# ruc-aimc-lab/GeoFormer

Measured on AMD Instinct MI355X. Metric: image-pairs/sec (640x640), higher is better.
Workload: dtype f16

## Files before the change

geoformer_amd/_lib.py:

```python
import ctypes
import os

_HERE = os.path.dirname(os.path.abspath(__file__))
LIB_PATH = os.environ.get('GF_LIB_PATH') or os.path.join(_HERE, 'libgeoformer_hip.so')

GF_F32, GF_F16, GF_BF16 = 0, 1, 2
GF_IMAGE_U8, GF_IMAGE_F32_NORMALISED, GF_IMAGE_F32_NORMALISED_RCP = 0, 1, 2

c_void_p, c_int, c_float, c_size_t = ctypes.c_void_p, ctypes.c_int, ctypes.c_float, ctypes.c_size_t
c_long, c_uint32 = ctypes.c_long, ctypes.c_uint32

SIGNATURES = {
    'gf_abi_version': (c_int, []),
    'gf_last_error': (ctypes.c_char_p, []),
    'gf_profile_filter': (None, [ctypes.c_char_p]),
    'gf_profile_enable': (None, [c_int]),
    'gf_profile_collect': (c_int, [ctypes.c_char_p, ctypes.POINTER(ctypes.c_double), ctypes.POINTER(c_int),
                                   ctypes.POINTER(ctypes.c_double)]),
    'gf_dual_softmax_workspace_bytes': (c_size_t, [c_int, c_int, c_int]),
    'gf_dual_softmax_match_only_supported': (c_int, [c_int, c_int, c_int, c_int, c_int, c_int]),
    'gf_dual_softmax_conf_at': (c_int, [c_void_p, c_void_p, c_int, c_int, c_int, c_int, c_int, c_float, c_void_p, c_void_p, c_void_p, c_int,
                                        c_void_p, c_void_p, c_size_t, c_void_p]),
    'gf_dual_softmax_match': (c_int, [c_void_p, c_void_p, c_int, c_int, c_int, c_int, c_int, c_void_p, c_void_p,
                                      c_float, c_float, c_int, c_int, c_int, c_float, c_void_p, c_void_p, c_void_p,
# ... 37 lines not shown
    'gf_encoder_kv_state': (c_int, [c_void_p, c_long, c_int, c_int, c_int, c_void_p, c_void_p, c_void_p, c_void_p, c_size_t, c_void_p]),
    'gf_encoder_layer': (c_int, [c_void_p, c_long, c_void_p, c_long, c_void_p, c_int, c_void_p, c_float, c_void_p, c_void_p, c_float,
                                 c_float, c_int, c_void_p, c_int, c_void_p, c_long, c_int, c_int, c_int, c_void_p]),
    'gf_encoder_layer_kv': (c_int, [c_void_p, c_long, c_void_p, c_int, c_void_p, c_float, c_void_p, c_void_p, c_float, c_float, c_int,
                                    c_void_p, c_long, c_int, c_int, c_int, c_void_p, c_int, c_void_p, c_void_p, c_size_t, c_void_p]),
    'gf_fine_layer': (c_int, [c_void_p, c_void_p, c_void_p, c_int, c_int, c_int, c_void_p, c_void_p, c_float, c_float, c_float, c_void_p]),
    'gf_conv3x3_supported': (c_int, [c_int, c_int]),
    'gf_conv3x3s2_supported': (c_int, [c_int, c_int]),
    'gf_lateral_supported': (c_int, [c_int, c_int]),
    'gf_lateral_upsample_add_nhwc': (c_int, [c_void_p, c_void_p, c_void_p, c_void_p, c_int, c_int, c_int, c_int, c_int, c_int, c_int, c_int, c_void_p]),
    'gf_conv3x3_nhwc': (c_int, [c_void_p, c_void_p, c_void_p, c_void_p, c_void_p, c_void_p, c_int, c_int, c_int, c_int, c_int, c_int,
                                c_float, c_int, c_void_p]),
    'gf_linear': (c_int, [c_void_p, c_long, c_int, c_void_p, c_long, c_int, c_void_p, c_void_p, c_void_p, c_int, c_int,
                          c_void_p, c_void_p, c_float, c_void_p, c_long, c_void_p, c_int, c_void_p, c_long, c_int, c_int,
                          c_int, c_void_p]),
    'gf_ransac_workspace_bytes': (c_size_t, [c_int, c_int]),
    'gf_ransac_homography': (c_int, [c_void_p, c_void_p, c_void_p, c_int, c_int, c_float, c_void_p, c_void_p, c_float,
                                     c_int, c_uint32, c_int, c_int, c_void_p, c_void_p, c_void_p, c_void_p, c_void_p, c_void_p,
                                     c_void_p, c_void_p, c_size_t, c_void_p]),
    'gf_ransac_homography_v2': (c_int, [c_void_p, c_void_p, c_void_p, c_int, c_int, c_float, c_void_p, c_void_p, c_float,
                                        c_int, c_uint32, c_int, c_int, c_void_p, c_void_p, c_void_p, c_void_p, c_void_p, c_void_p,
                                        c_void_p, c_void_p, c_size_t, c_void_p, c_int]),
    'gf_window_geometry': (c_int, [c_void_p, c_void_p, c_int, c_int, c_int, c_int, c_int, c_int, c_int, c_int,
                                   c_void_p, c_void_p, c_void_p, c_void_p, c_void_p]),
    'gf_inlier_index': (c_int, [c_void_p, c_void_p, c_void_p, c_void_p, c_int, c_int, c_int, c_int, c_int, c_int,
                                c_void_p, c_void_p, c_void_p, c_void_p, c_void_p, c_void_p]),
    'gf_self_attention_workspace_bytes': (c_size_t, [c_int, c_int, c_int]),
    'gf_self_attention_gathered': (c_int, [c_void_p, c_void_p, c_void_p, c_int, c_int, c_int, c_int, c_int, c_long,
                                           c_long, c_long, c_void_p, c_long, c_void_p, c_int, c_void_p, c_void_p,
                                           c_size_t, c_void_p]),
# ... 63 lines not shown
```

geoformer_amd/csrc/gf_common.h:

```cpp
#pragma once
#include <hip/hip_runtime.h>
#include <stdint.h>
#include <stdio.h>

#include "../../include/geoformer_hip.h"

typedef float v16f __attribute__((ext_vector_type(16)));
typedef float v4f __attribute__((ext_vector_type(4)));
typedef _Float16 v8h __attribute__((ext_vector_type(8)));
typedef _Float16 v4h __attribute__((ext_vector_type(4)));
typedef _Float16 v2h __attribute__((ext_vector_type(2)));
typedef uint32_t v4u __attribute__((ext_vector_type(4)));
typedef __bf16 gf_bf16;
typedef gf_bf16 v8b __attribute__((ext_vector_type(8)));
typedef gf_bf16 v4b __attribute__((ext_vector_type(4)));
template <typename T, int N>
using gf_vec = T __attribute__((ext_vector_type(N)));
typedef short gf_v4s __attribute__((__vector_size__(4 * sizeof(short))));

void gf_set_error(const char* fmt, ...);

#define GF_CHECK_ARG(cond, msg)                                   \
    do {                                                          \
        if (!(cond)) {                                            \
// ... 56 lines not shown
    static constexpr int kPer16B = 8;
};

__device__ __forceinline__ float gf_to_float(float x) { return x; }
__device__ __forceinline__ float gf_to_float(_Float16 x) { return (float)x; }
__device__ __forceinline__ float gf_to_float(gf_bf16 x) { return (float)x; }
template <typename T>
__device__ __forceinline__ T gf_from_float(float x);
template <>
__device__ __forceinline__ float gf_from_float<float>(float x) { return x; }
template <>
__device__ __forceinline__ _Float16 gf_from_float<_Float16>(float x) { return (_Float16)x; }
template <>
__device__ __forceinline__ gf_bf16 gf_from_float<gf_bf16>(float x) { return (gf_bf16)x; }

template <typename T>
struct Mma32;
template <>
struct Mma32<float> {
    using Frag = v4f;
    static constexpr int kGroup = 8;
    static __device__ __forceinline__ void mma(const Frag& a, const Frag& b, v16f& c) {
        c = __builtin_amdgcn_mfma_f32_32x32x2f32(a.x, b.x, c, 0, 0, 0);
        c = __builtin_amdgcn_mfma_f32_32x32x2f32(a.y, b.y, c, 0, 0, 0);
        c = __builtin_amdgcn_mfma_f32_32x32x2f32(a.z, b.z, c, 0, 0, 0);
        c = __builtin_amdgcn_mfma_f32_32x32x2f32(a.w, b.w, c, 0, 0, 0);
    }
};
template <>
struct Mma32<_Float16> {
// ... 138 lines not shown
```

geoformer_amd/csrc/k3_linear.hip:

```cpp
#include <math.h>

#include <type_traits>

#include "gf_common.h"

#ifndef K3_TRACE
#define K3_TRACE 0
#endif
#if K3_TRACE
__device__ long long k3_trace[1024 * 4 * 16];
#define K3_T(slot) do { if (lane == 0 && blockIdx.y == 0 && blockIdx.x < 1024) k3_trace[(blockIdx.x * 4 + wave) * 16 + (slot)] = clock64(); } while (0)
extern "C" int gf_debug_k3_trace(long long* out) {
    return (int)hipMemcpyFromSymbol(out, HIP_SYMBOL(k3_trace), sizeof(long long) * 1024 * 4 * 16);
}
#else
#define K3_T(slot)
#endif

namespace {

enum { EPI_NONE = 0, EPI_RELU = 1, EPI_TANH = 2, EPI_LN = 3, EPI_LN_RES = 4, EPI_UPADD = 5 };

struct LinArgs {
    const void* a1;
    const void* a2;
    long lda1, lda2;
    int k1, k2;
    const void* w;
    const float* bias;
    const void* rgbias;
    int rg_rows;
    const float* gamma;
    const float* beta;
    float eps;
    const void* res;
    long ldres;
    const int32_t* flag;
    int flag_rows;
    void* out;
    long ldo;
    int M, N;
    const void* up_lo;
    int up_h, up_w, up_H, up_W, up_n;
    float up_ry, up_rx;
    int rm_w;
    long rm_line, rm_pix;
};

__device__ __forceinline__ void lin_tile(int& row_tile, int& col_tile) {
    const int gx = gridDim.x, gy = gridDim.y;
    row_tile = blockIdx.x;
    col_tile = blockIdx.y;
    if (gy > 1 && (gx & 7) == 0) {
        const int id = blockIdx.y * gx + blockIdx.x, grp = id / (8 * gy), j = id - grp * (8 * gy);
        row_tile = grp * 8 + (j & 7);
        col_tile = j >> 3;
    }
}

template <typename T, int NB, int EPI, bool CONVX = false>
__global__ __launch_bounds__(256, sizeof(T) == 2 ? 2 : 1) void linear_kernel(LinArgs a) {
    using Mm = Mma32<T>;
    using Frag = typename Mm::Frag;
    constexpr int EPC = 16 / sizeof(T);
    constexpr int BK = 128 / sizeof(T);
    constexpr int WROWS = 32 * NB;
    constexpr int ROWS = 128 + WROWS;
    constexpr int NLD = ROWS * 8 / 256;
    extern __shared__ __attribute__((aligned(16))) char smem[];
    char* st = smem;
    char* sw = smem + 128 * 128;
    float* vec = reinterpret_cast<float*>(smem + ROWS * 128);
    const int tid = threadIdx.x, lane = tid & 63, wave = tid >> 6, h = lane >> 5, lr = lane & 31;
    int row_tile, col_tile;
    lin_tile(row_tile, col_tile);
    const int m0 = row_tile * 128, n0 = col_tile * WROWS;
    const int K = a.k1 + a.k2;
// ... 9 lines not shown
    int dst[NLD];
    bool isa[NLD];
#pragma unroll
    for (int p = 0; p < NLD; ++p) {
        const int e = p * 256 + tid, row = e >> 3, c = e & 7;
        isa[p] = row < 128;
        if (isa[p]) {
            src[p] = nullptr;
            dst[p] = gf_lds_off(row, c);
        } else {
            const int wr = row - 128;
            src[p] = (const T*)a.w + (size_t)min(n0 + wr, a.N - 1) * K + c * EPC;
            dst[p] = 128 * 128 + gf_lds_off(wr, c);
        }
    }
    v4u regs[NLD];
    const bool ragged = CONVX && (K % BK) != 0;
    auto gload = [&](int k0) {
        const bool first = k0 < a.k1;
        const T* ab = (const T*)(first ? a.a1 : a.a2);
        const long ld = first ? a.lda1 : a.lda2;
        const int kk = first ? k0 : k0 - a.k1;
#pragma unroll
        for (int p = 0; p < NLD; ++p) {
            const int e = p * 256 + tid, row = e >> 3, c = e & 7;
            const T* g;
            if (isa[p]) {
                const int r = min(m0 + row, a.M - 1);
                const size_t ro = (CONVX && a.rm_w > 0) ? (size_t)(r / a.rm_w) * a.rm_line + (size_t)(r % a.rm_w) * a.rm_pix : (size_t)r * ld;
                g = ab + ro + kk + c * EPC;
            } else {
                g = src[p] + k0;
            }
            if (!ragged || k0 + c * EPC < K) regs[p] = *reinterpret_cast<const v4u*>(g);
            else regs[p] = v4u{0u, 0u, 0u, 0u};
        }
    };
    auto lstore = [&]() {
#pragma unroll
        for (int p = 0; p < NLD; ++p) *reinterpret_cast<v4u*>(smem + dst[p]) = regs[p];
    };
// ... 216 lines not shown
        for (int nb = 0; nb < NB; ++nb)
#pragma unroll
            for (int r4 = 0; r4 < 4; ++r4) {
                const int c = nb * 32 + 8 * r4 + 4 * h;
                if (n0 + c >= a.N) continue;
                v4f v{acc[nb][4 * r4], acc[nb][4 * r4 + 1], acc[nb][4 * r4 + 2], acc[nb][4 * r4 + 3]};
                if constexpr (EPI == EPI_LN_RES) {
                    const v4f x = *reinterpret_cast<const v4f*>(rp + c);
                    v = keep ? v4f{x.x + v.x, x.y + v.y, x.z + v.z, x.w + v.w} : x;
                }
                *reinterpret_cast<v4f*>(op + c) = v;
            }
    }
}

template <typename T, int EPI>
__global__ __launch_bounds__(256, 2) void linear_kernel_w2(LinArgs a) {
    using Frag = typename Mma32<T>::Frag;
    using V4 = gf_vec<T, 4>;
    using V8 = gf_vec<T, 8>;
    constexpr int EPC = 8, BK = 64, WROWS = 256, ROWS = 128 + WROWS, NLD = ROWS * 8 / 256;
    extern __shared__ __attribute__((aligned(16))) char smem[];
    char* st = smem;
    char* sw = smem + 128 * 128;
    float* vec = reinterpret_cast<float*>(smem + ROWS * 128);
    const int tid = threadIdx.x, lane = tid & 63, wave = tid >> 6, h = lane >> 5, lr = lane & 31;
    const int tm = wave >> 1, tn = wave & 1;
    int row_tile, col_tile;
    lin_tile(row_tile, col_tile);
    const int m0 = row_tile * 128, n0 = col_tile * WROWS;
    const int K = a.k1 + a.k2;
    if (tid < WROWS) vec[tid] = (a.bias && n0 + tid < a.N) ? a.bias[n0 + tid] : 0.f;
    const T* src[NLD];
    int dst[NLD];
    bool isa[NLD];
#pragma unroll
    for (int p = 0; p < NLD; ++p) {
        const int e = p * 256 + tid, row = e >> 3, c = e & 7;
        isa[p] = row < 128;
        if (isa[p]) {
            src[p] = nullptr;
            dst[p] = gf_lds_off(row, c);
        } else {
            const int wr = row - 128;
            src[p] = (const T*)a.w + (size_t)min(n0 + wr, a.N - 1) * K + c * EPC;
            dst[p] = 128 * 128 + gf_lds_off(wr, c);
        }
    }
    v4u regs[NLD];
    auto gload = [&](int k0) {
        const bool first = k0 < a.k1;
        const T* ab = (const T*)(first ? a.a1 : a.a2);
        const long ld = first ? a.lda1 : a.lda2;
        const int kk = first ? k0 : k0 - a.k1;
#pragma unroll
        for (int p = 0; p < NLD; ++p) {
            const int e = p * 256 + tid, row = e >> 3, c = e & 7;
            const T* g = isa[p] ? ab + (size_t)min(m0 + row, a.M - 1) * ld + kk + c * EPC : src[p] + k0;
            regs[p] = *reinterpret_cast<const v4u*>(g);
        }
    };
    v16f acc[2][4];
#pragma unroll
    for (int t = 0; t < 2; ++t)
#pragma unroll
        for (int nb = 0; nb < 4; ++nb)
#pragma unroll
            for (int r = 0; r < 16; ++r) acc[t][nb][r] = 0.f;
    const int nk = K / BK;
    gload(0);
    for (int kt = 0; kt < nk; ++kt) {
        __syncthreads();
// ... 33 lines not shown
    for (int t = 0; t < 2; ++t) {
#pragma unroll
        for (int nb = 0; nb < 4; ++nb)
#pragma unroll
            for (int r4 = 0; r4 < 4; ++r4) {
                const int c = nb * 32 + 8 * r4 + 4 * h;
                *reinterpret_cast<V4*>(ot + lr * RS + c * 2) =
                    V4{(T)acc[t][nb][4 * r4], (T)acc[t][nb][4 * r4 + 1], (T)acc[t][nb][4 * r4 + 2], (T)acc[t][nb][4 * r4 + 3]};
            }
        __builtin_amdgcn_fence(__ATOMIC_RELEASE, "wavefront");
        __builtin_amdgcn_wave_barrier();
        __builtin_amdgcn_fence(__ATOMIC_ACQUIRE, "wavefront");
#pragma unroll
        for (int it = 0; it < 8; ++it) {
            const int row = it * 4 + prow, tg = m0 + tm * 64 + t * 32 + row, cg = n0 + tn * 128 + pch * 8;
            if (tg >= a.M || cg >= a.N) continue;
            *reinterpret_cast<V8*>((T*)a.out + (size_t)tg * a.ldo + cg) = *reinterpret_cast<const V8*>(ot + row * RS + pch * 16);
        }
        __builtin_amdgcn_fence(__ATOMIC_RELEASE, "wavefront");
        __builtin_amdgcn_wave_barrier();
    }
}

template <typename T, int NB, int EPI, bool CONVX = false>
void lin_launch1(const LinArgs& a, hipStream_t st) {
    constexpr int WROWS = 32 * NB;
    size_t lds = (size_t)(128 + WROWS) * 128 + 3 * WROWS * sizeof(float);
    if (lds < 4 * 32 * 272) lds = 4 * 32 * 272;
    linear_kernel<T, NB, EPI, CONVX><<<dim3((a.M + 127) / 128, (a.N + WROWS - 1) / WROWS), 256, lds, st>>>(a);
}

template <typename T, int NB>
void lin_launch(const LinArgs& a, int epi, hipStream_t st) {
    switch (epi) {
        case EPI_NONE: lin_launch1<T, NB, EPI_NONE>(a, st); break;
        case EPI_RELU: lin_launch1<T, NB, EPI_RELU>(a, st); break;
        case EPI_TANH: lin_launch1<T, NB, EPI_TANH>(a, st); break;
        case EPI_LN: lin_launch1<T, NB, EPI_LN>(a, st); break;
        default: lin_launch1<T, NB, EPI_LN_RES>(a, st); break;
    }
}

}

// ... 42 lines not shown
    } else if (dtype == GF_F32) {
        if (wide) lin_launch<float, 8>(a, epilogue, st);
        else lin_launch<float, 4>(a, epilogue, st);
    } else if (dtype == GF_F16) {
        if (wide) lin_launch<_Float16, 8>(a, epilogue, st);
        else lin_launch<_Float16, 4>(a, epilogue, st);
    } else {
        if (wide) lin_launch<gf_bf16, 8>(a, epilogue, st);
        else lin_launch<gf_bf16, 4>(a, epilogue, st);
    }
    gf_prof_end("k3_linear", pt, st);
    GF_CHECK_LAUNCH();
    return GF_OK;
}

extern "C" int gf_conv1x1_upsample_add_nhwc(const void* x, const void* w, const void* lo, void* out, int N, int h, int wl,
                                            int H, int W, int Cin, int Cout, int dtype, void* stream) {
    GF_CHECK_ARG(x && w && lo && out, "null pointer");
    GF_CHECK_ARG(N > 0 && h > 0 && wl > 0 && H > 0 && W > 0, "empty problem");
    GF_CHECK_ARG(dtype == GF_F16 || dtype == GF_BF16, "built for 16-bit maps (the inference backbone)");
    GF_CHECK_ARG(Cin % 32 == 0 && Cout % 32 == 0, "Cin and Cout must be multiples of 32");
    GF_CHECK_ARG((long)N * H * W < (1l << 31), "too many pixels");
    GF_CHECK_ARG((uintptr_t)x % 16 == 0 && (uintptr_t)out % 16 == 0 && (uintptr_t)lo % 16 == 0, "tensors must be 16-byte aligned");
    LinArgs a{};
    a.a1 = x; a.lda1 = Cin; a.k1 = Cin; a.w = w; a.out = out; a.ldo = Cout; a.M = N * H * W; a.N = Cout;
    a.up_lo = lo; a.up_h = h; a.up_w = wl; a.up_H = H; a.up_W = W; a.up_n = N;
    a.up_ry = H > 1 ? (float)(h - 1) / (float)(H - 1) : 0.f;
    a.up_rx = W > 1 ? (float)(wl - 1) / (float)(W - 1) : 0.f;
    hipStream_t st = (hipStream_t)stream;
    void* pt = gf_prof_begin("k3_upadd", st, 2.0 * ((double)a.M * (Cin + Cout) + (double)N * h * wl * Cout + (double)Cin * Cout));
// ... 29 lines not shown
```

geoformer_amd/csrc/k_fine.hip:

```cpp
#include <math.h>

#include <type_traits>

#include "gf_common.h"

namespace {

struct FgArgs {
    const void* f0;
    const void* f1;
    long s0n, s0c, s0h, s0w, s1n, s1c, s1h, s1w;
    int H0, W0, H1, W1, C;
    const void* c0;
    const void* c1;
    int L, S, CC;
    const int64_t* b_ids;
    const int64_t* i_ids;
    const int64_t* j_ids;
    int M, w0c, w1c, stride, W;
    void* win;
    void* ccat;
};

template <typename TF, typename T>
// ... 6 lines not shown
    const TF* f = (const TF*)(side ? a.f1 : a.f0);
    const long sn = side ? a.s1n : a.s0n, sc = side ? a.s1c : a.s0c, sh = side ? a.s1h : a.s0h, sw = side ? a.s1w : a.s0w;
    const int cy = (cell / wc) * a.stride - a.W / 2, cx = (cell % wc) * a.stride - a.W / 2;
    T* out = (T*)a.win + ((size_t)side * a.M + m) * a.W * a.W * a.C;
    if (t < a.C) {
        for (int k = 0; k < a.W * a.W; ++k) {
            const int y = cy + k / a.W, x = cx + k % a.W;
            float v = 0.f;
            if (y >= 0 && y < Hf && x >= 0 && x < Wf) v = gf_to_float(f[b * sn + t * sc + y * sh + x * sw]);
            out[(size_t)k * a.C + t] = gf_from_float<T>(v);
        }
    }
    const T* cf = (const T*)(side ? a.c1 : a.c0) + ((size_t)b * (side ? a.S : a.L) + cell) * a.CC;
    T* co = (T*)a.ccat + ((size_t)side * a.M + m) * a.CC;
    for (int c = t; c < a.CC; c += blockDim.x) co[c] = cf[c];
}

template <typename TF, typename T>
__device__ __forceinline__ v4u fg_convert8(v4u v) {
    if constexpr (std::is_same<TF, T>::value) {
        return v;
    } else {
        const gf_vec<TF, 8> x = __builtin_bit_cast(gf_vec<TF, 8>, v);
        gf_vec<T, 8> o;
#pragma unroll
        for (int k = 0; k < 8; ++k) o[k] = gf_from_float<T>(gf_to_float(x[k]));
        return __builtin_bit_cast(v4u, o);
    }
}

template <typename TF, typename T>
__global__ __launch_bounds__(256) void fine_gather_rows(FgArgs a) {
    static_assert(sizeof(TF) == 2 && sizeof(T) == 2, "16-byte pieces of 8 elements on both sides");
    const int lane = threadIdx.x & 63, u = blockIdx.x * 4 + (threadIdx.x >> 6);
    if (u >= 2 * a.M) return;
    const int side = u >= a.M, m = side ? u - a.M : u;
    const int b = (int)a.b_ids[m];
    const int cell = (int)(side ? a.j_ids[m] : a.i_ids[m]);
    const int wc = side ? a.w1c : a.w0c;
    const int Hf = side ? a.H1 : a.H0, Wf = side ? a.W1 : a.W0;
    const TF* f = (const TF*)(side ? a.f1 : a.f0);
    const long sn = side ? a.s1n : a.s0n, sh = side ? a.s1h : a.s0h, sw = side ? a.s1w : a.s0w;
    const int cy = (cell / wc) * a.stride - a.W / 2, cx = (cell % wc) * a.stride - a.W / 2;
// ... 307 lines not shown
```

geoformer_amd/model/modules.py:

```python
import copy
import math
from typing import Dict, Optional

import torch
import torch.nn as nn
from .. import fused, ops


class PositionEncodingSine(nn.Module):

    def __init__(self, d_model, max_shape=(256, 256), temp_bug_fix=False):
        super().__init__()
        self.d_model, self.max_shape, self.temp_bug_fix = d_model, tuple(max_shape), temp_bug_fix
        self._tables = {}

    def table(self, h, w, device):
        key = (h, w, str(device))
        if key not in self._tables:
            if h > self.max_shape[0] or w > self.max_shape[1]:
                raise ValueError(f'feature map {h}x{w} exceeds max_shape {self.max_shape}')
            c = self.d_model
            ypos = torch.ones(h, w).cumsum(0).float().unsqueeze(0)
            xpos = torch.ones(h, w).cumsum(1).float().unsqueeze(0)
            k2 = torch.arange(0, c // 2, 2).float()
# ... 61 lines not shown
    def fusable_window(self, dtype, seq_len):
        return (dtype != torch.float32 and self.d_model == 128 and self.nhead == 8 and self.attention_kind == 'linear'
                and self.activation == 'relu' and seq_len <= 32)

    def invalidate(self):
        self._cache = {}

    def project_q(self, x):
        return ops.linear(x, self.weights(x.dtype)['q'])

    def project_kv(self, source):
        kv = ops.linear(source, self.weights(source.dtype)['kv'])
        c = self.d_model
        return kv[..., :c], kv[..., c:]

    def project_qkv(self, x):
        qkv = ops.linear(x, self.weights(x.dtype)['qkv'])
        c = self.d_model
        return qkv[..., :c], qkv[..., c:2 * c], qkv[..., 2 * c:]

    def finish(self, x, message, row_flag=None, flag_rows=0, out=None):
        w = self.weights(x.dtype)
        if self.fusable(x.dtype):
            return fused.encoder_layer(x, w['stream_finish'], w['ln'], self.norm1.eps, self.norm2.eps,
                                       0 if self.activation == 'relu' else 1, msg=message, row_flag=row_flag,
                                       flag_rows=flag_rows, out=out)
        act = ops.EPI_RELU if self.activation == 'relu' else ops.EPI_TANH
        message = ops.linear(message, w['merge'], epilogue=ops.EPI_LN, ln=w['n1'], eps=self.norm1.eps)
        hid = ops.linear(x, w['w1'], a2=message, epilogue=act)
        return ops.linear(hid, w['w2'], epilogue=ops.EPI_LN_RES, ln=w['n2'], eps=self.norm2.eps, residual=x,
# ... 201 lines not shown
    return out


class GeoTransformer(nn.Module):
    def __init__(self, config, layer_names, d_model, linear=True):
        super().__init__()
        if linear:
            raise NotImplementedError('GeoModule builds its transformer with linear=False (geo_module.py:20-21)')
        self.config, self.d_model, self.layer_names, self.nhead = config, d_model, layer_names, config['nhead']
        layer = LoFTREncoderLayer(d_model, self.nhead, 'full', 'tanh')
        self.layers = nn.ModuleList([copy.deepcopy(layer) for _ in self.layer_names])
        for p in self.parameters():
            if p.dim() > 1:
                nn.init.xavier_uniform_(p)
        self.norm = nn.LayerNorm(d_model)

    def forward(self, feat0, feat1, geo, both: Optional[torch.Tensor] = None):
        assert self.d_model == feat0.size(2), 'the feature number of src and transformer must be equal'
        n, L, S = feat0.shape[0], feat0.shape[1], feat1.shape[1]
        same = feat0.shape == feat1.shape
        nk = geo['nidx']
        if same:
            if both is None:
                both = torch.cat([feat0, feat1], 0)
            feat0, feat1 = both[:n], both[n:]
        for layer, name in zip(self.layers, self.layer_names):
            if name == 'self':
                if same:
                    q, k, v = layer.project_qkv(both)
                    msg = ops.self_attention_gathered(q, k, v, geo['idx_both'], geo['nidx_both'], self.nhead)
                    both = layer.finish(both, msg, geo['nidx_both'], L)
                    feat0, feat1 = both[:n], both[n:]
                else:
                    k, v = layer.project_kv(feat0)
                    m0 = ops.self_attention_gathered(layer.project_q(feat0), k, v, geo['idx0'], nk[:, 0], self.nhead)
                    k, v = layer.project_kv(feat1)
                    m1 = ops.self_attention_gathered(layer.project_q(feat1), k, v, geo['idx1'], nk[:, 1], self.nhead)
                    feat0 = layer.finish(feat0, m0, geo['nidx_t'][0], L)
                    feat1 = layer.finish(feat1, m1, geo['nidx_t'][1], S)
            elif name == 'cross':
                if same:
                    q, k, v = layer.project_qkv(both)
                    q0, q1, k0, k1, v0, v1 = q[:n], q[n:], k[:n], k[n:], v[:n], v[n:]
                else:
                    k0, v0 = layer.project_kv(feat0)
                    k1, v1 = layer.project_kv(feat1)
                    q0, q1 = layer.project_q(feat0), layer.project_q(feat1)
                m0 = ops.window_cross_attention(q0, k1, v1, geo['win1'], geo['valid'], self.nhead, geo.get('hw0'), geo.get('hw1'))
                m1 = ops.window_cross_attention(q1, k0, v0, geo['win0'], geo['valid'], self.nhead, geo.get('hw1'), geo.get('hw0'))
                if same:
                    nxt = torch.empty_like(both)
                    layer.finish(feat0, m0, geo['valid'], L, out=nxt[:n])
# ... 108 lines not shown
                 'db': self.down_proj.bias.detach().float().contiguous(),
                 'mw_win': mw[:, :d].to(dtype).contiguous(), 'mw_ctx': mw[:, d:].to(dtype).contiguous(),
                 'mb': self.merge_feat.bias.detach().float().contiguous()}
            self._cache[dtype] = w
        return w

    def forward(self, feat_f0, feat_f1, feat_c0, feat_c1, data: Dict[str, torch.Tensor]):
        W = self.W
        stride = int(data['hw0_f'][0]) // int(data['hw0_c'][0])
        data.update({'W': torch.tensor(W)})
        dtype = feat_c0.dtype
        M = data['b_ids'].shape[0]
        if M == 0:
            e = torch.empty(0, W ** 2, self.d_model_f, device=feat_f0.device, dtype=dtype)
            return e, e.clone()
        win, ccat = ops.fine_gather(feat_f0, feat_f1, feat_c0, feat_c1, data['b_ids'], data['i_ids'], data['j_ids'],
                                    int(data['hw0_c'][1]), int(data['hw1_c'][1]), stride, W, dtype)
        w = self.weights(dtype)
        ctx = ops.linear(ops.linear(ccat, w['dw'], bias=w['db']), w['mw_ctx'], bias=w['mb'])
        out = ops.linear(win, w['mw_win'], rowgroup_bias=ctx, rowgroup_rows=W * W)
        return out[:M], out[M:]


class FineMatching2(nn.Module):
    def __init__(self, temperature=0.1, thr=0.1):
        super().__init__()
        self.temperature, self.thr = temperature, thr

    def forward(self, feat_f0, feat_f1, data: Dict[str, torch.Tensor]):
        M, WW, C = feat_f0.shape
        if M == 0:
            data.update({'fine_matrix': torch.empty(0, WW, WW, device=feat_f0.device),
                         'mkpts0_f': data['mkpts0_c'], 'mkpts1_f': data['mkpts1_c']})
# ... 8 lines not shown
```

geoformer_amd/ops.py:

```python
import ctypes

import torch

from . import _lib
from ._lib import GF_BF16, GF_F16, GF_F32, check

_DTYPES = {torch.float32: GF_F32, torch.float16: GF_F16, torch.bfloat16: GF_BF16}


def _dt(t):
    try:
        return _DTYPES[t.dtype]
    except KeyError:
        raise TypeError(f'geoformer_amd kernels take float32, float16 or bfloat16 tensors, got {t.dtype}') from None


def _p(t):
    return None if t is None else ctypes.c_void_p(t.data_ptr())


_raw_stream = getattr(torch._C, '_cuda_getCurrentRawStream', None)
_raw_device = getattr(torch._C, '_cuda_getDevice', None)


# ... 462 lines not shown
    if a2 is not None:
        a2, lda2 = _rows2d(a2)
        k2 = a2.shape[-1]
    N = w.shape[0]
    M = a1.numel() // k1
    if out is None:
        out = torch.empty(*a1.shape[:-1], N, dtype=a1.dtype, device=a1.device)
    elif out.shape != (*a1.shape[:-1], N) or out.dtype != a1.dtype or not out.is_contiguous():
        raise ValueError('out must be a contiguous tensor of the result shape and dtype')
    res, ldres = (None, 0) if residual is None else _rows2d(residual)
    g, b = (None, None) if ln is None else ln
    check(_lib.lib().gf_linear(_p(a1), lda1, k1, _p(a2), lda2, k2, _p(w), _p(bias), _p(rowgroup_bias), int(rowgroup_rows),
                               int(epilogue), _p(g), _p(b), float(eps), _p(res), ldres, _p(row_flag), int(flag_rows), _p(out),
                               N, _dt(a1), M, N, _stream()), 'gf_linear')
    return out


class CoarseFocalLoss(torch.autograd.Function):

    @staticmethod
    def forward(ctx, f0, f1, pos_b, pos_i, pos_j, temperature, alpha, gamma, weight, mask0=None, mask1=None):
        _need_cuda(f0, f1, pos_b)
        N, L, C = f0.shape
        S = f1.shape[1]
        P = pos_b.numel()
        ctx_dtype = f0.dtype
        if f0.dtype == torch.bfloat16:
            f0, f1 = f0.to(torch.float16), f1.to(torch.float16)
        f0c, f1c = _contig(f0), _contig(f1)
        if f0c.dtype not in (torch.float32, torch.float16) or f1c.dtype != f0c.dtype:
# ... 173 lines not shown
```

include/geoformer_hip.h:

```cpp
#ifndef GEOFORMER_HIP_H_
#define GEOFORMER_HIP_H_

#include <stddef.h>
#include <stdint.h>

#ifdef __cplusplus
extern "C" {
#endif

typedef enum { GF_OK = 0, GF_ERR_INVALID_ARGUMENT = -1, GF_ERR_WORKSPACE = -2, GF_ERR_LAUNCH = -3 } gf_status;
typedef enum { GF_F32 = 0, GF_F16 = 1, GF_BF16 = 2 } gf_dtype;

#define GF_ABI_VERSION 4
int gf_abi_version(void);
const char* gf_last_error(void);

void gf_profile_enable(int on);
void gf_profile_filter(const char* tag);
int gf_profile_collect(const char* tag, double* total_ms, int* count, double* work);

size_t gf_dual_softmax_workspace_bytes(int N, int L, int S);
int gf_dual_softmax_match_only_supported(int dtype, int L, int S, int C, int masked, int force_one);
int gf_dual_softmax_conf_at(const void* f0, const void* f1, int dtype, int N, int L, int S, int C, float temperature,
                            const int64_t* b, const int64_t* i, const int64_t* j, int P, float* out, void* workspace,
// ... 72 lines not shown

#define GF_CONV_PAD16 0x100
#define GF_CONV_REM8 0x200
#define GF_CONV_S2 0x400
int gf_conv3x3_supported(int cin, int cout);
int gf_conv3x3s2_supported(int cin, int cout);
int gf_conv3x3_nhwc(const void* x, const void* wstream, const float* shift, const void* residual, void* out,
                    const void* zeros, int N, int H, int W, int cin, int cout, int act, float slope, int dtype,
                    void* stream);

int gf_linear(const void* a1, long lda1, int k1, const void* a2, long lda2, int k2, const void* w,
              const float* bias, const void* rowgroup_bias, int rowgroup_rows, int epilogue,
              const float* ln_gamma, const float* ln_beta, float ln_eps, const void* residual, long ldres,
              const int32_t* row_flag, int flag_rows, void* out, long ldo, int dtype, int M, int N,
              void* stream);

size_t gf_ransac_workspace_bytes(int N, int iters);
int gf_ransac_homography(const float* mkpts0_c, const float* mkpts1_c, const int32_t* counts, int N,
                         int capacity, float scale, const float* scale0, const float* scale1, float thr,
                         int iters, uint32_t seed, int min_points, int integer_keypoints, float* kp0, float* kp1, double* M,
                         float* M_f32, float* Minv_f32, int32_t* valid, uint8_t* keep, void* workspace,
                         size_t workspace_bytes, void* stream);
int gf_ransac_homography_v2(const float* mkpts0_c, const float* mkpts1_c, const int32_t* counts, int N,
                            int capacity, float scale, const float* scale0, const float* scale1, float thr,
                            int iters, uint32_t seed, int min_points, int integer_keypoints, float* kp0, float* kp1, double* M,
                            float* M_f32, float* Minv_f32, int32_t* valid, uint8_t* keep, void* workspace,
                            size_t workspace_bytes, void* stream, int lm_iters);

int gf_window_geometry(const float* H, const int32_t* valid, int N, int hq, int wq, int Himg, int Wimg,
                       int wk, int scale, int window_size, const float* window_scale, int32_t* win,
// ... 67 lines not shown
```

Before: 732.1.

## Fuse row gathers and fine window extraction into linear GEMM loads

Adds a gathered-row variant of the two-block linear kernel so self-attention K/V projections are computed only on the rows each sample actually attends to. It also adds a window-gathering linear that reads fine-level feature windows straight from the maps inside the GEMM load, removing the separate fine_gather pass and its intermediate buffer. The model paths switch to these for 16-bit inputs. Per-row address computation and scattered loads add overhead. The gathered self-attention path also changes how queries index keys, which could cost more if counts are close to full.

```diff
diff --git a/geoformer_amd/_lib.py b/geoformer_amd/_lib.py
--- a/geoformer_amd/_lib.py
+++ b/geoformer_amd/_lib.py
@@ -75,6 +75,11 @@
     'gf_linear': (c_int, [c_void_p, c_long, c_int, c_void_p, c_long, c_int, c_void_p, c_void_p, c_void_p, c_int, c_int,
                           c_void_p, c_void_p, c_float, c_void_p, c_long, c_void_p, c_int, c_void_p, c_long, c_int, c_int,
                           c_int, c_void_p]),
+    'gf_linear_rows': (c_int, [c_void_p, c_long, c_int, c_int, c_void_p, c_long, c_void_p, c_int, c_void_p, c_void_p, c_void_p, c_long,
+                               c_int, c_int, c_int, c_int, c_void_p]),
+    'gf_linear_windows': (c_int, [c_void_p, c_void_p, c_int, c_void_p, c_void_p, c_int, c_int, c_int, c_int, c_int, c_void_p, c_void_p,
+                                  c_void_p, c_int, c_int, c_int, c_int, c_int, c_void_p, c_void_p, c_void_p, c_void_p, c_int, c_int,
+                                  c_void_p]),
     'gf_ransac_workspace_bytes': (c_size_t, [c_int, c_int]),
     'gf_ransac_homography': (c_int, [c_void_p, c_void_p, c_void_p, c_int, c_int, c_float, c_void_p, c_void_p, c_float,
                                      c_int, c_uint32, c_int, c_int, c_void_p, c_void_p, c_void_p, c_void_p, c_void_p, c_void_p,
diff --git a/geoformer_amd/csrc/gf_common.h b/geoformer_amd/csrc/gf_common.h
--- a/geoformer_amd/csrc/gf_common.h
+++ b/geoformer_amd/csrc/gf_common.h
@@ -2,6 +2,8 @@
 #include <hip/hip_runtime.h>
 #include <stdint.h>
 #include <stdio.h>
+
+#include <type_traits>
 
 #include "../../include/geoformer_hip.h"
 
@@ -94,6 +96,19 @@
 template <>
 __device__ __forceinline__ gf_bf16 gf_from_float<gf_bf16>(float x) { return (gf_bf16)x; }
 
+template <typename TF, typename T>
+__device__ __forceinline__ v4u fg_convert8(v4u v) {
+    if constexpr (std::is_same<TF, T>::value) {
+        return v;
+    } else {
+        const gf_vec<TF, 8> x = __builtin_bit_cast(gf_vec<TF, 8>, v);
+        gf_vec<T, 8> o;
+#pragma unroll
+        for (int k = 0; k < 8; ++k) o[k] = gf_from_float<T>(gf_to_float(x[k]));
+        return __builtin_bit_cast(v4u, o);
+    }
+}
+
 template <typename T>
 struct Mma32;
 template <>
diff --git a/geoformer_amd/csrc/k3_linear.hip b/geoformer_amd/csrc/k3_linear.hip
--- a/geoformer_amd/csrc/k3_linear.hip
+++ b/geoformer_amd/csrc/k3_linear.hip
@@ -3,6 +3,7 @@
 #include <type_traits>
 
 #include "gf_common.h"
+#include "k3_rowmap.h"
 
 #ifndef K3_TRACE
 #define K3_TRACE 0
@@ -20,6 +21,17 @@
 namespace {
 
 enum { EPI_NONE = 0, EPI_RELU = 1, EPI_TANH = 2, EPI_LN = 3, EPI_LN_RES = 4, EPI_UPADD = 5 };
+
+struct FwArgs {
+    const void* f0;
+    const void* f1;
+    long s0n, s0h, s0w, s1n, s1h, s1w;
+    int H0, W0, H1, W1;
+    const int64_t* b_ids;
+    const int64_t* i_ids;
+    const int64_t* j_ids;
+    int M, w0c, w1c, stride, W;
+};
 
 struct LinArgs {
     const void* a1;
@@ -45,6 +57,11 @@
     float up_ry, up_rx;
     int rm_w;
     long rm_line, rm_pix;
+    const int32_t* gr_idx;
+    const int32_t* gr_cnt;
+    long gr_idx_ld;
+    int gr_cnt_ld, gr_cap, gr_src;
+    FwArgs fw;
 };
 
 __device__ __forceinline__ void lin_tile(int& row_tile, int& col_tile) {
@@ -58,9 +75,10 @@
     }
 }
 
-template <typename T, int NB, int EPI, bool CONVX = false>
+template <typename T, int NB, int EPI, bool CONVX = false, typename TF = void>
 __global__ __launch_bounds__(256, sizeof(T) == 2 ? 2 : 1) void linear_kernel(LinArgs a) {
     using Mm = Mma32<T>;
+    constexpr bool FW = !std::is_void<TF>::value;
     using Frag = typename Mm::Frag;
     constexpr int EPC = 16 / sizeof(T);
     constexpr int BK = 128 / sizeof(T);
@@ -100,6 +118,23 @@
             dst[p] = 128 * 128 + gf_lds_off(wr, c);
         }
     }
+    using TFE = std::conditional_t<FW, TF, T>;
+    [[maybe_unused]] const TFE* fwp[FW ? NLD : 1];
+    if constexpr (FW) {
+        const FwArgs& f = a.fw;
+        const int ww = f.W * f.W;
+#pragma unroll
+        for (int p = 0; p < NLD; ++p) {
+            fwp[p] = nullptr;
+            if (!isa[p]) continue;
+            const int e = p * 256 + tid, r = min(m0 + (e >> 3), a.M - 1), u = r / ww, k = r - u * ww;
+            const bool side = u >= f.M;
+            const int m = side ? u - f.M : u, b = (int)f.b_ids[m], cell = (int)(side ? f.j_ids[m] : f.i_ids[m]), wc = side ? f.w1c : f.w0c;
+            const int y = (cell / wc) * f.stride - f.W / 2 + k / f.W, x = (cell % wc) * f.stride - f.W / 2 + k % f.W;
+            if (y >= 0 && y < (side ? f.H1 : f.H0) && x >= 0 && x < (side ? f.W1 : f.W0))
+                fwp[p] = (const TFE*)(side ? f.f1 : f.f0) + b * (side ? f.s1n : f.s0n) + y * (side ? f.s1h : f.s0h) + x * (side ? f.s1w : f.s0w) + (e & 7) * EPC;
+        }
+    }
     v4u regs[NLD];
     const bool ragged = CONVX && (K % BK) != 0;
     auto gload = [&](int k0) {
@@ -111,6 +146,12 @@
         for (int p = 0; p < NLD; ++p) {
             const int e = p * 256 + tid, row = e >> 3, c = e & 7;
             const T* g;
+            if constexpr (FW) {
+                if (isa[p]) {
+                    regs[p] = fwp[p] ? fg_convert8<TFE, T>(*reinterpret_cast<const v4u*>(fwp[p] + k0)) : v4u{0u, 0u, 0u, 0u};
+                    continue;
+                }
+            }
             if (isa[p]) {
                 const int r = min(m0 + row, a.M - 1);
                 const size_t ro = (CONVX && a.rm_w > 0) ? (size_t)(r / a.rm_w) * a.rm_line + (size_t)(r % a.rm_w) * a.rm_pix : (size_t)r * ld;
@@ -357,7 +398,7 @@
     }
 }
 
-template <typename T, int EPI>
+template <typename T, int EPI, bool GATHER = false>
 __global__ __launch_bounds__(256, 2) void linear_kernel_w2(LinArgs a) {
     using Frag = typename Mma32<T>::Frag;
     using V4 = gf_vec<T, 4>;
@@ -371,12 +412,24 @@
     const int tm = wave >> 1, tn = wave & 1;
     int row_tile, col_tile;
     lin_tile(row_tile, col_tile);
-    const int m0 = row_tile * 128, n0 = col_tile * WROWS;
+    int m0 = row_tile * 128, mlim = a.M;
+    const int n0 = col_tile * WROWS;
+    size_t orow0 = 0;
+    const int32_t* gidx = nullptr;
+    if constexpr (GATHER) {
+        const int tps = (a.gr_cap + 127) / 128, s = row_tile / tps;
+        m0 = (row_tile - s * tps) * 128;
+        mlim = min(max(a.gr_cnt[(size_t)s * a.gr_cnt_ld], 0), a.gr_cap);
+        if (m0 >= mlim) return;
+        orow0 = (size_t)s * a.gr_cap;
+        gidx = a.gr_idx + (size_t)s * a.gr_idx_ld;
+    }
     const int K = a.k1 + a.k2;
     if (tid < WROWS) vec[tid] = (a.bias && n0 + tid < a.N) ? a.bias[n0 + tid] : 0.f;
     const T* src[NLD];
     int dst[NLD];
     bool isa[NLD];
+    [[maybe_unused]] int avo[GATHER ? NLD : 1];
 #pragma unroll
     for (int p = 0; p < NLD; ++p) {
         const int e = p * 256 + tid, row = e >> 3, c = e & 7;
@@ -384,11 +437,20 @@
         if (isa[p]) {
             src[p] = nullptr;
             dst[p] = gf_lds_off(row, c);
+            if constexpr (GATHER) {
+                const int ix = m0 + row < mlim ? gidx[m0 + row] : -1;
+                avo[p] = (unsigned)ix < (unsigned)a.gr_src ? ix * (int)(a.lda1 * sizeof(T)) + c * 16 : GF_ROWMAP_OOB;
+            }
         } else {
             const int wr = row - 128;
             src[p] = (const T*)a.w + (size_t)min(n0 + wr, a.N - 1) * K + c * EPC;
             dst[p] = 128 * 128 + gf_lds_off(wr, c);
         }
+    }
+    [[maybe_unused]] GfRsrc ars;
+    if constexpr (GATHER) {
+        const int s = (int)(orow0 / (size_t)a.gr_cap);
+        ars = gf_rsrc((const T*)a.a1 + (size_t)s * a.gr_src * a.lda1, (unsigned)((size_t)a.gr_src * a.lda1 * sizeof(T)));
     }
     v4u regs[NLD];
     auto gload = [&](int k0) {
@@ -399,6 +461,12 @@
 #pragma unroll
         for (int p = 0; p < NLD; ++p) {
             const int e = p * 256 + tid, row = e >> 3, c = e & 7;
+            if constexpr (GATHER) {
+                if (isa[p]) {
+                    regs[p] = __builtin_bit_cast(v4u, __builtin_amdgcn_raw_buffer_load_b128(ars.r, avo[p] + k0 * (int)sizeof(T), 0, 0));
+                    continue;
+                }
+            }
             const T* g = isa[p] ? ab + (size_t)min(m0 + row, a.M - 1) * ld + kk + c * EPC : src[p] + k0;
             regs[p] = *reinterpret_cast<const v4u*>(g);
         }
@@ -462,20 +530,20 @@
 #pragma unroll
         for (int it = 0; it < 8; ++it) {
             const int row = it * 4 + prow, tg = m0 + tm * 64 + t * 32 + row, cg = n0 + tn * 128 + pch * 8;
-            if (tg >= a.M || cg >= a.N) continue;
-            *reinterpret_cast<V8*>((T*)a.out + (size_t)tg * a.ldo + cg) = *reinterpret_cast<const V8*>(ot + row * RS + pch * 16);
+            if (tg >= mlim || cg >= a.N) continue;
+            *reinterpret_cast<V8*>((T*)a.out + (orow0 + tg) * a.ldo + cg) = *reinterpret_cast<const V8*>(ot + row * RS + pch * 16);
         }
         __builtin_amdgcn_fence(__ATOMIC_RELEASE, "wavefront");
         __builtin_amdgcn_wave_barrier();
     }
 }
 
-template <typename T, int NB, int EPI, bool CONVX = false>
+template <typename T, int NB, int EPI, bool CONVX = false, typename TF = void>
 void lin_launch1(const LinArgs& a, hipStream_t st) {
     constexpr int WROWS = 32 * NB;
     size_t lds = (size_t)(128 + WROWS) * 128 + 3 * WROWS * sizeof(float);
     if (lds < 4 * 32 * 272) lds = 4 * 32 * 272;
-    linear_kernel<T, NB, EPI, CONVX><<<dim3((a.M + 127) / 128, (a.N + WROWS - 1) / WROWS), 256, lds, st>>>(a);
+    linear_kernel<T, NB, EPI, CONVX, TF><<<dim3((a.M + 127) / 128, (a.N + WROWS - 1) / WROWS), 256, lds, st>>>(a);
 }
 
 template <typename T, int NB>
@@ -548,6 +616,66 @@
     return GF_OK;
 }
 
+extern "C" int gf_linear_rows(const void* a, long lda, int k, int src_rows, const int32_t* row_idx, long idx_stride,
+                              const int32_t* row_count, int count_stride, const void* w, const float* bias, void* out, long ldo,
+                              int dtype, int samples, int cap, int N, void* stream) {
+    GF_CHECK_ARG(a && row_idx && row_count && w && out, "null pointer");
+    GF_CHECK_ARG(dtype == GF_F16 || dtype == GF_BF16, "built for 16-bit storage");
+    GF_CHECK_ARG(k > 0 && k % 64 == 0, "k must be a multiple of 64");
+    GF_CHECK_ARG(N > 0 && N % 256 == 0, "N must be a multiple of 256");
+    GF_CHECK_ARG(idx_stride >= 0 && count_stride >= 0, "negative stride");
+    GF_CHECK_ARG((lda * 2) % 16 == 0 && (uintptr_t)a % 16 == 0, "operand rows must be 16-byte aligned");
+    GF_CHECK_ARG((ldo * 2) % 16 == 0 && (uintptr_t)out % 16 == 0 && ldo >= N, "output rows must be 16-byte aligned");
+    GfRowmapPlan plan;
+    const char* why = gf_rowmap_plan(samples, cap, src_rows, lda, k, 2, &plan);
+    GF_CHECK_ARG(why == nullptr, why);
+    LinArgs la{};
+    la.a1 = a; la.lda1 = lda; la.k1 = k; la.w = w; la.bias = bias; la.out = out; la.ldo = ldo; la.M = samples * cap; la.N = N;
+    la.gr_idx = row_idx; la.gr_cnt = row_count; la.gr_idx_ld = idx_stride; la.gr_cnt_ld = count_stride; la.gr_cap = cap; la.gr_src = src_rows;
+    hipStream_t st = (hipStream_t)stream;
+    void* pt = gf_prof_begin("k3_linear_rows", st, 0.0);
+    const size_t lds = (size_t)(128 + 256) * 128 + 256 * sizeof(float);
+    const dim3 grid(plan.grid_x, N / 256);
+    if (dtype == GF_F16) linear_kernel_w2<_Float16, EPI_NONE, true><<<grid, 256, lds, st>>>(la);
+    else linear_kernel_w2<gf_bf16, EPI_NONE, true><<<grid, 256, lds, st>>>(la);
+    gf_prof_end("k3_linear_rows", pt, st);
+    GF_CHECK_LAUNCH();
+    return GF_OK;
+}
+
+extern "C" int gf_linear_windows(const void* feat0, const void* feat1, int feat_dtype, const long* strides0, const long* strides1,
+                                 int H0, int W0, int H1, int W1, int C, const int64_t* b_ids, const int64_t* i_ids,
+                                 const int64_t* j_ids, int M, int w0c, int w1c, int stride, int window, const void* w,
+                                 const float* bias, const void* rowgroup_bias, void* out, int dtype, int N, void* stream) {
+    GF_CHECK_ARG(feat0 && feat1 && strides0 && strides1 && b_ids && i_ids && j_ids && w && out, "null pointer");
+    GF_CHECK_ARG((dtype == GF_F16 || dtype == GF_BF16) && (feat_dtype == GF_F16 || feat_dtype == GF_BF16), "built for 16-bit storage");
+    GF_CHECK_ARG(dtype == feat_dtype || (feat_dtype == GF_BF16 && dtype == GF_F16), "maps of the output type, or bf16 maps with fp16 output");
+    GF_CHECK_ARG(H0 > 0 && W0 > 0 && H1 > 0 && W1 > 0 && w0c > 0 && w1c > 0 && stride > 0, "bad sizes");
+    GF_CHECK_ARG(C > 0 && C % 64 == 0, "C must be a multiple of 64");
+    GF_CHECK_ARG(N > 0 && N % 128 == 0, "N must be a multiple of 128");
+    GF_CHECK_ARG(strides0[1] == 1 && strides1[1] == 1, "channels-last maps");
+    GF_CHECK_ARG((uintptr_t)feat0 % 16 == 0 && (uintptr_t)feat1 % 16 == 0 && (uintptr_t)out % 16 == 0 && (uintptr_t)w % 16 == 0,
+                 "tensors must be 16-byte aligned");
+    for (int d = 0; d < 4; ++d)
+        GF_CHECK_ARG(d == 1 || (strides0[d] % 8 == 0 && strides1[d] % 8 == 0), "pixel rows must be 16-byte aligned");
+    int rows = 0;
+    const char* why = gf_window_rows(M, window, &rows);
+    GF_CHECK_ARG(why == nullptr, why);
+    LinArgs la{};
+    la.a1 = feat0; la.k1 = C; la.w = w; la.bias = bias; la.rgbias = rowgroup_bias; la.rg_rows = window * window;
+    la.out = out; la.ldo = N; la.M = rows; la.N = N;
+    la.fw = FwArgs{feat0, feat1, strides0[0], strides0[2], strides0[3], strides1[0], strides1[2], strides1[3], H0, W0, H1, W1,
+                   b_ids, i_ids, j_ids, M, w0c, w1c, stride, window};
+    hipStream_t st = (hipStream_t)stream;
+    void* pt = gf_prof_begin("k3_linear_windows", st, 2.0 * ((double)rows * (C + N) + (double)N * C + (rowgroup_bias ? 2.0 * M * N : 0.0)));
+    if (dtype == GF_BF16) lin_launch1<gf_bf16, 4, EPI_NONE, false, gf_bf16>(la, st);
+    else if (feat_dtype == GF_F16) lin_launch1<_Float16, 4, EPI_NONE, false, _Float16>(la, st);
+    else lin_launch1<_Float16, 4, EPI_NONE, false, gf_bf16>(la, st);
+    gf_prof_end("k3_linear_windows", pt, st);
+    GF_CHECK_LAUNCH();
+    return GF_OK;
+}
+
 extern "C" int gf_conv1x1_upsample_add_nhwc(const void* x, const void* w, const void* lo, void* out, int N, int h, int wl,
                                             int H, int W, int Cin, int Cout, int dtype, void* stream) {
     GF_CHECK_ARG(x && w && lo && out, "null pointer");
diff --git a/geoformer_amd/csrc/k3_rowmap.h b/geoformer_amd/csrc/k3_rowmap.h
--- /dev/null
+++ b/geoformer_amd/csrc/k3_rowmap.h
@@ -0,0 +1,34 @@
+#pragma once
+#include <stdint.h>
+
+constexpr int GF_ROWMAP_OOB = 0x7FFF0000;
+
+struct GfRowmapPlan {
+    int tiles_per_sample;
+    int grid_x;
+    uint32_t source_bytes;
+};
+
+inline const char* gf_rowmap_plan(long samples, long cap, long src_rows, long lda, long k, int elem_bytes, GfRowmapPlan* p) {
+    if (samples <= 0 || cap <= 0 || src_rows <= 0 || k <= 0 || elem_bytes <= 0) return "empty problem";
+    if (lda < k) return "row stride shorter than a row";
+    if (lda > (1l << 24) || src_rows > (1l << 31) - 1 || cap > (1l << 31) - 1 || samples > (1l << 31) - 1) return "shape too large";
+    if ((long)k * elem_bytes > 0xFFFF) return "rows too long";
+    const int64_t bytes = (int64_t)src_rows * lda * elem_bytes;
+    if (bytes > (int64_t)GF_ROWMAP_OOB) return "a sample's source rows exceed the 2 GiB a row map addresses";
+    const int64_t tiles = (cap + 127) / 128, gx = tiles * samples;
+    if (gx > 0x7FFFFFFFll || (int64_t)samples * cap > 0x7FFFFFFFll) return "too many rows";
+    p->tiles_per_sample = (int)tiles;
+    p->grid_x = (int)gx;
+    p->source_bytes = (uint32_t)bytes;
+    return nullptr;
+}
+
+inline const char* gf_window_rows(long matches, long window, int* rows) {
+    if (matches <= 0 || window <= 0) return "empty problem";
+    if (window > 64) return "window too large";
+    const int64_t per_match = 2 * (int64_t)window * window;
+    if (matches > (0x7FFFFFFFll - 128) / per_match) return "too many window rows";
+    *rows = (int)(matches * per_match);
+    return nullptr;
+}
diff --git a/geoformer_amd/csrc/k_fine.hip b/geoformer_amd/csrc/k_fine.hip
--- a/geoformer_amd/csrc/k_fine.hip
+++ b/geoformer_amd/csrc/k_fine.hip
@@ -44,19 +44,6 @@
     const T* cf = (const T*)(side ? a.c1 : a.c0) + ((size_t)b * (side ? a.S : a.L) + cell) * a.CC;
     T* co = (T*)a.ccat + ((size_t)side * a.M + m) * a.CC;
     for (int c = t; c < a.CC; c += blockDim.x) co[c] = cf[c];
-}
-
-template <typename TF, typename T>
-__device__ __forceinline__ v4u fg_convert8(v4u v) {
-    if constexpr (std::is_same<TF, T>::value) {
-        return v;
-    } else {
-        const gf_vec<TF, 8> x = __builtin_bit_cast(gf_vec<TF, 8>, v);
-        gf_vec<T, 8> o;
-#pragma unroll
-        for (int k = 0; k < 8; ++k) o[k] = gf_from_float<T>(gf_to_float(x[k]));
-        return __builtin_bit_cast(v4u, o);
-    }
 }
 
 template <typename TF, typename T>
diff --git a/geoformer_amd/model/modules.py b/geoformer_amd/model/modules.py
--- a/geoformer_amd/model/modules.py
+++ b/geoformer_amd/model/modules.py
@@ -99,6 +99,11 @@
         c = self.d_model
         return kv[..., :c], kv[..., c:]
 
+    def project_kv_rows(self, source, row_idx, row_count):
+        kv = ops.linear_rows(source, self.weights(source.dtype)['kv'], row_idx, row_count)
+        c = self.d_model
+        return kv[..., :c], kv[..., c:]
+
     def project_qkv(self, x):
         qkv = ops.linear(x, self.weights(x.dtype)['qkv'])
         c = self.d_model
@@ -330,6 +335,20 @@
             if p.dim() > 1:
                 nn.init.xavier_uniform_(p)
         self.norm = nn.LayerNorm(d_model)
+        self._identity = {}
+
+    def _identity_index(self, n, rows, device):
+        t = self._identity.get((rows, device))
+        if t is None:
+            t = self._identity[(rows, device)] = torch.arange(rows, dtype=torch.int32, device=device)
+        return t.expand(n, rows)
+
+    def _self_message(self, layer, x, idx, nkeys):
+        if x.dtype == torch.float32:
+            q, k, v = layer.project_qkv(x)
+            return ops.self_attention_gathered(q, k, v, idx, nkeys, self.nhead)
+        k, v = layer.project_kv_rows(x, idx, nkeys)
+        return ops.self_attention_gathered(layer.project_q(x), k, v, self._identity_index(x.shape[0], x.shape[1], x.device), nkeys, self.nhead)
 
     def forward(self, feat0, feat1, geo, both: Optional[torch.Tensor] = None):
         assert self.d_model == feat0.size(2), 'the feature number of src and transformer must be equal'
@@ -343,15 +362,12 @@
         for layer, name in zip(self.layers, self.layer_names):
             if name == 'self':
                 if same:
-                    q, k, v = layer.project_qkv(both)
-                    msg = ops.self_attention_gathered(q, k, v, geo['idx_both'], geo['nidx_both'], self.nhead)
+                    msg = self._self_message(layer, both, geo['idx_both'], geo['nidx_both'])
                     both = layer.finish(both, msg, geo['nidx_both'], L)
                     feat0, feat1 = both[:n], both[n:]
                 else:
-                    k, v = layer.project_kv(feat0)
-                    m0 = ops.self_attention_gathered(layer.project_q(feat0), k, v, geo['idx0'], nk[:, 0], self.nhead)
-                    k, v = layer.project_kv(feat1)
-                    m1 = ops.self_attention_gathered(layer.project_q(feat1), k, v, geo['idx1'], nk[:, 1], self.nhead)
+                    m0 = self._self_message(layer, feat0, geo['idx0'], nk[:, 0])
+                    m1 = self._self_message(layer, feat1, geo['idx1'], nk[:, 1])
                     feat0 = layer.finish(feat0, m0, geo['nidx_t'][0], L)
                     feat1 = layer.finish(feat1, m1, geo['nidx_t'][1], S)
             elif name == 'cross':
@@ -490,9 +506,14 @@
         if M == 0:
             e = torch.empty(0, W ** 2, self.d_model_f, device=feat_f0.device, dtype=dtype)
             return e, e.clone()
-        win, ccat = ops.fine_gather(feat_f0, feat_f1, feat_c0, feat_c1, data['b_ids'], data['i_ids'], data['j_ids'],
-                                    int(data['hw0_c'][1]), int(data['hw1_c'][1]), stride, W, dtype)
         w = self.weights(dtype)
+        ids = (data['b_ids'], data['i_ids'], data['j_ids'])
+        w0c, w1c = int(data['hw0_c'][1]), int(data['hw1_c'][1])
+        if ops.fine_windows_16bit(feat_f0, feat_f1, dtype):
+            ctx = ops.linear(ops.linear_coarse_rows(feat_c0, feat_c1, *ids, w['dw'], bias=w['db']), w['mw_ctx'], bias=w['mb'])
+            out = ops.linear_windows(feat_f0, feat_f1, *ids, w0c, w1c, stride, W, w['mw_win'], dtype, rowgroup_bias=ctx)
+            return out[:M], out[M:]
+        win, ccat = ops.fine_gather(feat_f0, feat_f1, feat_c0, feat_c1, *ids, w0c, w1c, stride, W, dtype)
         ctx = ops.linear(ops.linear(ccat, w['dw'], bias=w['db']), w['mw_ctx'], bias=w['mb'])
         out = ops.linear(win, w['mw_win'], rowgroup_bias=ctx, rowgroup_rows=W * W)
         return out[:M], out[M:]
diff --git a/geoformer_amd/ops.py b/geoformer_amd/ops.py
--- a/geoformer_amd/ops.py
+++ b/geoformer_amd/ops.py
@@ -500,6 +500,62 @@
                                int(epilogue), _p(g), _p(b), float(eps), _p(res), ldres, _p(row_flag), int(flag_rows), _p(out),
                                N, _dt(a1), M, N, _stream()), 'gf_linear')
     return out
+
+
+def linear_rows(a, w, row_idx, row_count, cap=None, bias=None, out=None):
+    _need_cuda(a, w, row_idx, row_count)
+    S, R, K = a.shape
+    a, lda = _rows2d(a)
+    if a.stride(0) != lda * R:
+        raise ValueError('linear_rows needs batch stride == rows * row stride')
+    cap = R if cap is None else int(cap)
+    N = w.shape[0]
+    if row_idx.dtype != torch.int32 or row_count.dtype != torch.int32 or row_idx.shape[0] != S or row_idx.shape[1] < cap or row_idx.stride(1) != 1:
+        raise ValueError('row_idx must be int32 [S, >= cap] with contiguous rows, row_count int32')
+    if row_count.numel() != S:
+        raise ValueError('row_count must hold one entry per sample')
+    if out is None:
+        out = torch.empty(S, cap, N, dtype=a.dtype, device=a.device)
+    elif out.shape != (S, cap, N) or out.dtype != a.dtype or not out.is_contiguous():
+        raise ValueError('out must be a contiguous tensor of the result shape and dtype')
+    check(_lib.lib().gf_linear_rows(_p(a), lda, K, R, _p(row_idx), row_idx.stride(0), _p(row_count), row_count.stride(0) if row_count.dim() else 1,
+                                    _p(w), _p(bias), _p(out), N, _dt(a), S, cap, N, _stream()), 'gf_linear_rows')
+    return out
+
+
+def fine_windows_16bit(feat_f0, feat_f1, out_dtype):
+    ok = (torch.float16, torch.bfloat16)
+    if feat_f0.dtype not in ok or feat_f1.dtype != feat_f0.dtype or out_dtype not in ok:
+        return False
+    if feat_f0.dtype != out_dtype and not (feat_f0.dtype == torch.bfloat16 and out_dtype == torch.float16):
+        return False
+    return all(f.stride(1) == 1 and f.data_ptr() % 16 == 0 and all(f.stride(d) % 8 == 0 for d in (0, 2, 3)) for f in (feat_f0, feat_f1))
+
+
+def linear_windows(feat0, feat1, b_ids, i_ids, j_ids, w0c, w1c, stride, window, w, out_dtype, bias=None, rowgroup_bias=None):
+    _need_cuda(feat0, feat1, b_ids, w)
+    M, C, N = b_ids.shape[0], feat0.shape[1], w.shape[0]
+    if w.dtype != out_dtype or w.shape[1] != C or not w.is_contiguous():
+        raise ValueError('linear_windows: w must be a contiguous [N, C] tensor of out_dtype')
+    if rowgroup_bias is not None and (rowgroup_bias.shape != (2 * M, N) or rowgroup_bias.dtype != out_dtype or not rowgroup_bias.is_contiguous()):
+        raise ValueError('linear_windows: rowgroup_bias must be a contiguous [2M, N] tensor of out_dtype')
+    out = torch.empty(2 * M, window * window, N, dtype=out_dtype, device=feat0.device)
+    s0 = (ctypes.c_long * 4)(*feat0.stride())
+    s1 = (ctypes.c_long * 4)(*feat1.stride())
+    check(_lib.lib().gf_linear_windows(_p(feat0), _p(feat1), _dt(feat0), ctypes.cast(s0, ctypes.c_void_p), ctypes.cast(s1, ctypes.c_void_p),
+                                       feat0.shape[2], feat0.shape[3], feat1.shape[2], feat1.shape[3], C, _p(_contig(b_ids)),
+                                       _p(_contig(i_ids)), _p(_contig(j_ids)), M, int(w0c), int(w1c), int(stride), int(window), _p(w),
+                                       _p(bias), _p(rowgroup_bias), _p(out), _DTYPES[out_dtype], N, _stream()), 'gf_linear_windows')
+    return out
+
+
+def linear_coarse_rows(feat_c0, feat_c1, b_ids, i_ids, j_ids, w, bias=None):
+    def as_map(f):
+        f = _contig(f)
+        n, rows, cc = f.shape
+        return f.as_strided((n, cc, 1, rows), (rows * cc, 1, rows * cc, cc))
+    m0, m1 = as_map(feat_c0), as_map(feat_c1)
+    return linear_windows(m0, m1, b_ids, i_ids, j_ids, m0.shape[3], m1.shape[3], 1, 1, w, feat_c0.dtype, bias=bias)[:, 0]
 
 
 class CoarseFocalLoss(torch.autograd.Function):
diff --git a/include/geoformer_hip.h b/include/geoformer_hip.h
--- a/include/geoformer_hip.h
+++ b/include/geoformer_hip.h
@@ -110,6 +110,15 @@
               const float* ln_gamma, const float* ln_beta, float ln_eps, const void* residual, long ldres,
               const int32_t* row_flag, int flag_rows, void* out, long ldo, int dtype, int M, int N,
               void* stream);
+
+int gf_linear_rows(const void* a, long lda, int k, int src_rows, const int32_t* row_idx, long idx_stride,
+                   const int32_t* row_count, int count_stride, const void* w, const float* bias, void* out, long ldo,
+                   int dtype, int samples, int cap, int N, void* stream);
+
+int gf_linear_windows(const void* feat0, const void* feat1, int feat_dtype, const long* strides0, const long* strides1,
+                      int H0, int W0, int H1, int W1, int C, const int64_t* b_ids, const int64_t* i_ids,
+                      const int64_t* j_ids, int M, int w0c, int w1c, int stride, int window, const void* w,
+                      const float* bias, const void* rowgroup_bias, void* out, int dtype, int N, void* stream);
 
 size_t gf_ransac_workspace_bytes(int N, int iters);
 int gf_ransac_homography(const float* mkpts0_c, const float* mkpts1_c, const int32_t* counts, int N,
```

New measurement: 739.2, median of 6. About the same (+1.0%).
